# mravanelli/pytorch-kaldi

Hardware: AMD Instinct MI355X
Metric: train_frames_per_sec (higher is better)
Workload: dtype bf16

## Files before the change

include/pk_amd.h:

```cpp
#ifndef PK_AMD_H
#define PK_AMD_H

#include <stdint.h>

#ifdef __cplusplus
extern "C" {
#endif

#define PK_PREC_F32 0
#define PK_PREC_BF16 1

#define PK_ACT_LINEAR 0
#define PK_ACT_RELU 1
#define PK_ACT_TANH 2
#define PK_ACT_SIGMOID 3
#define PK_ACT_LEAKY_RELU 4
#define PK_ACT_ELU 5

#define PK_CELL_LIGRU 0
#define PK_CELL_RNN 1
#define PK_CELL_LSTM 2
#define PK_CELL_GRU 3
#define PK_CELL_MINGRU 4

// ... 152 lines not shown
                         float mask_scalar, const float* ln_gamma, float ln_eps, const float* Y, const float* S,
                         const float* LNS, const float* dY, uint16_t* dGb, int64_t g_pitch, int prefilled, float* lnwork,
                         float* dln_gamma, float* dln_beta);
unsigned pk_persist2_error_count(void);
void pk_persist2_error_reset(void);

int pk_conv1d_pool_fwd(void* stream, const float* x, const float* w, const float* bias, int B, int Cin, int L,
                       int Cout, int K, int pool, float* y, int32_t* argmax, float* work);
int64_t pk_conv_fwd_work_floats(int Cin, int Cout, int K);
int64_t pk_conv_partial_floats(int B, int Cin, int L, int Cout, int K, int pool);
int pk_conv1d_pool_bwd(void* stream, const float* x, const float* w, const float* dy, const int32_t* argmax, int B,
                       int Cin, int L, int Cout, int K, int pool, float* dw, float* dbias, float* dx,
                       float* partial);

int pk_rmsprop_step(void* stream, float* p, const float* g, float* square_avg, int64_t n, float lr, float alpha,
                    float eps, float weight_decay);
int pk_sgd_step(void* stream, float* p, const float* g, float* momentum_buf, int64_t n, float lr, float momentum,
                float weight_decay, int first_step);
int pk_adam_step(void* stream, float* p, const float* g, float* exp_avg, float* exp_avg_sq, float* max_exp_avg_sq,
                 int64_t n, float lr, float beta1, float beta2, float eps, float weight_decay, int step);
int pk_fused_step(void* stream, int kind, float* p, float* g, float* s0, float* s1, float* s2, int64_t n, float lr, float h0,
                  float h1, float h2, float weight_decay, int step, int zero_grad, const int64_t* segs, int nseg,
                  uint16_t* shadow);

unsigned pk_persist_error_count(void);
void pk_persist_error_reset(void);

int pk_linear_bn_act_bf16_covers(int64_t M, int64_t N, int64_t K);
int pk_linear_bn_act_bf16(void* stream, int M, int N, int K, const uint16_t* xb, int64_t ldx, const uint16_t* wb, int64_t ldw,
                          const float* bias, const float* gamma, const float* beta, float eps, float momentum,
                          float* running_mean, float* running_var, int act, const float* mask, float* z, float* a,
                          float* y, uint16_t* yb, int64_t ldyb, float* mean, float* var);
int pk_gemm_bf16_small_splitk(int M, int N, int K);
int pk_linear_bn_act_bf16_sk(void* stream, int M, int N, int K, const uint16_t* xb, int64_t ldx, const uint16_t* wb,
                             int64_t ldw, const float* bias, const float* gamma, const float* beta, float eps,
                             float momentum, float* running_mean, float* running_var, int act, const float* mask,
                             float* z, float* a, float* y, uint16_t* yb, int64_t ldyb, float* mean, float* var,
                             int splitk, float* ws);
int pk_conv1d_pool_dgrad(void* stream, const float* w, const float* dy, const int32_t* argmax, int B, int Cin, int L, int Cout,
                         int K, int pool, float* dx, float* work);
int pk_conv_bf16_covers(int Cin, int Cout, int K, int pool);
int64_t pk_conv_bf16_work_floats(int B, int Cin, int L, int Cout, int K, int pool, int backward);
int pk_conv1d_pool_fwd_bf16(void* stream, const float* x, const float* w, const float* bias, int B, int Cin, int L, int Cout,
                            int K, int pool, float* y, int32_t* argmax, float* work);
int pk_conv1d_pool_bwd_bf16(void* stream, const float* x, const float* w, const float* dy, const int32_t* argmax, int B,
                            int Cin, int L, int Cout, int K, int pool, float* dw, float* dx, float* work);
// ... 21 lines not shown
```

pytorch-kaldi_amd/_lib.py:

```python
import ctypes
import os
import re
import threading

HERE = os.path.dirname(os.path.abspath(__file__))
LIB_PATH = os.path.join(HERE, "lib", "libpk_amd.so")
HEADER = os.path.join(HERE, "..", "include", "pk_amd.h")

_lock = threading.Lock()
_lib = None

c_void_p, c_int, c_float, c_double, c_int64 = ctypes.c_void_p, ctypes.c_int, ctypes.c_float, ctypes.c_double, ctypes.c_int64
P = c_void_p

SIGNATURES = {
    "pk_version": (c_int, []),
    "pk_last_error": (ctypes.c_char_p, []),
    "pk_num_cu": (c_int, []),
    "pk_gemm": (c_int, [P, c_int, c_int, c_int, c_int, c_float, P, c_int64, c_int64, P, c_int64, c_int64, c_float, P,
                        c_int64, P, c_int, P]),
    "pk_gemm_f32_set_form": (None, [c_int]),
    "pk_gemm_bf16_tile_m": (c_int, [c_int]),
    "pk_gemm_bf16_auto_splitk": (c_int, [c_int, c_int, c_int]),
    "pk_gemm_bf16_set_tile": (None, [c_int]),
# ... 76 lines not shown
    "pk_persist2_set_lstm_waves": (None, [c_int]),
    "pk_rec_helper_set_mode": (None, [c_int]),
    "pk_rec_helper_get_mode": (c_int, []),
    "pk_persist2_get_lstm_waves": (c_int, []),
    "pk_persist2_error_count": (ctypes.c_uint, []),
    "pk_persist2_error_reset": (None, []),
    "pk_conv1d_pool_fwd": (c_int, [P, P, P, P, c_int, c_int, c_int, c_int, c_int, c_int, P, P, P]),
    "pk_conv_fwd_work_floats": (c_int64, [c_int, c_int, c_int]),
    "pk_conv_partial_floats": (c_int64, [c_int, c_int, c_int, c_int, c_int, c_int]),
    "pk_conv1d_pool_bwd": (c_int, [P, P, P, P, P, c_int, c_int, c_int, c_int, c_int, c_int, P, P, P, P]),
    "pk_ark_open": (P, [ctypes.c_char_p, c_int64]),
    "pk_ark_close": (None, [P]),
    "pk_ark_next": (c_int, [P, c_int, ctypes.c_char_p, c_int, ctypes.POINTER(c_int64), ctypes.POINTER(c_int64)]),
    "pk_ark_read": (c_int, [P, P]),
    "pk_ark_skip": (c_int, [P]),
    "pk_ivec_next": (c_int, [P, ctypes.c_char_p, c_int, ctypes.POINTER(c_int64)]),
    "pk_ivec_read": (c_int, [P, P]),
    "pk_context_window": (c_int, [P, c_int64, c_int64, c_int, c_int, P]),
    "pk_mean_var_norm": (c_int, [P, c_int64, c_int64]),
    "pk_rmsprop_step": (c_int, [P, P, P, P, c_int64, c_float, c_float, c_float, c_float]),
    "pk_sgd_step": (c_int, [P, P, P, P, c_int64, c_float, c_float, c_float, c_int]),
    "pk_adam_step": (c_int, [P, P, P, P, P, P, c_int64, c_float, c_float, c_float, c_float, c_float, c_int]),
    "pk_fused_step": (c_int, [P, c_int, P, P, P, P, P, c_int64, c_float, c_float, c_float, c_float, c_float, c_int, c_int, P, c_int, P]),
    "pk_persist_error_count": (ctypes.c_uint, []),
    "pk_persist_error_reset": (None, []),
    "pk_linear_bn_act_bf16_covers": (c_int, [c_int64, c_int64, c_int64]),
    "pk_linear_bn_act_bf16": (c_int, [P, c_int, c_int, c_int, P, c_int64, P, c_int64, P, P, P, c_float, c_float, P, P, c_int, P,
                                      P, P, P, P, c_int64, P, P]),
    "pk_gemm_bf16_small_splitk": (c_int, [c_int, c_int, c_int]),
    "pk_linear_bn_act_bf16_sk": (c_int, [P, c_int, c_int, c_int, P, c_int64, P, c_int64, P, P, P, c_float, c_float, P, P, c_int, P,
                                         P, P, P, P, c_int64, P, P, c_int, P]),
    "pk_selftest_mfma": (c_int, [P, ctypes.POINTER(c_int)]),
    "pk_selftest_permlane": (c_int, [P, ctypes.POINTER(c_int)]),
    "pk_selftest_dpp_row_sum": (c_int, [P, ctypes.POINTER(c_int)]),
    "pk_selftest_cu_hog": (c_int, [P, c_int, c_int, P]),
}


def declared_symbols():
    with open(HEADER) as f:
        text = re.sub(r"/\*.*?\*/", "", f.read(), flags=re.S)
    return sorted(set(re.findall(r"\b(pk_[a-z0-9_]+)\s*\(", text)))


class PkError(RuntimeError):
    pass
# ... 199 lines not shown
```

pytorch-kaldi_amd/csrc/pk_optim.hip:

```cpp
#include "pk_common.h"

namespace {

__global__ void rmsprop_kernel(float* __restrict__ p, const float* __restrict__ g, float* __restrict__ sq, long n, float lr,
                               float alpha, float eps, float wd) {
    for (long i = blockIdx.x * (long)blockDim.x + threadIdx.x; i < n; i += (long)gridDim.x * blockDim.x) {
        float gv = g[i];
        const float pv = p[i];
        if (wd != 0.f) gv += wd * pv;
        const float s = alpha * sq[i] + (1.f - alpha) * gv * gv;
        sq[i] = s;
        p[i] = pv - lr * gv / (sqrtf(s) + eps);
    }
}

__global__ void sgd_kernel(float* __restrict__ p, const float* __restrict__ g, float* __restrict__ buf, long n, float lr,
                           float momentum, float wd, int first) {
    for (long i = blockIdx.x * (long)blockDim.x + threadIdx.x; i < n; i += (long)gridDim.x * blockDim.x) {
        float gv = g[i];
        const float pv = p[i];
        if (wd != 0.f) gv += wd * pv;
        if (momentum != 0.f) {
            const float b = first ? gv : momentum * buf[i] + gv;
            buf[i] = b;
// ... 3 lines not shown
    }
}

__global__ void adam_kernel(float* __restrict__ p, const float* __restrict__ g, float* __restrict__ m, float* __restrict__ v,
                            float* __restrict__ vmax, long n, float lr, float beta1, float beta2, float eps, float wd,
                            float bc1, float bc2s) {
    for (long i = blockIdx.x * (long)blockDim.x + threadIdx.x; i < n; i += (long)gridDim.x * blockDim.x) {
        float gv = g[i];
        const float pv = p[i];
        if (wd != 0.f) gv += wd * pv;
        const float mv = beta1 * m[i] + (1.f - beta1) * gv;
        float vv = beta2 * v[i] + (1.f - beta2) * gv * gv;
        m[i] = mv;
        v[i] = vv;
        if (vmax != nullptr) {
            vv = fmaxf(vmax[i], vv);
            vmax[i] = vv;
        }
        const float denom = sqrtf(vv) / bc2s + eps;
        p[i] = pv - (lr / bc1) * (mv / denom);
    }
}

template <int KIND>
__global__ void fused_step_kernel(float* __restrict__ p, float* __restrict__ g, float* __restrict__ s0, float* __restrict__ s1,
                                  float* __restrict__ s2, long n, float lr, float h0, float h1, float h2, float wd, float bc1,
                                  float bc2s, int first, int zero_grad, const long* __restrict__ segs, int nseg,
                                  unsigned short* __restrict__ shadow) {
    for (long i = 4 * (blockIdx.x * (long)blockDim.x + threadIdx.x); i < n; i += 4 * (long)gridDim.x * blockDim.x) {
        f32x4 gv = *reinterpret_cast<const f32x4*>(g + i);
        f32x4 pv = *reinterpret_cast<const f32x4*>(p + i);
        if (wd != 0.f) {
#pragma unroll
            for (int e = 0; e < 4; ++e) gv[e] += wd * pv[e];
        }
        if (KIND == 0) {
            f32x4 sq = *reinterpret_cast<const f32x4*>(s0 + i);
#pragma unroll
            for (int e = 0; e < 4; ++e) {
                sq[e] = h0 * sq[e] + (1.f - h0) * gv[e] * gv[e];
                pv[e] = pv[e] - lr * gv[e] / (sqrtf(sq[e]) + h1);
            }
            *reinterpret_cast<f32x4*>(s0 + i) = sq;
        } else if (KIND == 1) {
            if (h0 != 0.f) {
                f32x4 b = *reinterpret_cast<const f32x4*>(s0 + i);
#pragma unroll
// ... 7 lines not shown
            for (int e = 0; e < 4; ++e) pv[e] = pv[e] - lr * gv[e];
        } else {
            f32x4 m = *reinterpret_cast<const f32x4*>(s0 + i), v = *reinterpret_cast<const f32x4*>(s1 + i);
            f32x4 vm = v;
#pragma unroll
            for (int e = 0; e < 4; ++e) {
                m[e] = h0 * m[e] + (1.f - h0) * gv[e];
                v[e] = h1 * v[e] + (1.f - h1) * gv[e] * gv[e];
                vm[e] = v[e];
            }
            *reinterpret_cast<f32x4*>(s0 + i) = m;
            *reinterpret_cast<f32x4*>(s1 + i) = v;
            if (s2 != nullptr) {
                const f32x4 old = *reinterpret_cast<const f32x4*>(s2 + i);
#pragma unroll
                for (int e = 0; e < 4; ++e) vm[e] = fmaxf(old[e], v[e]);
                *reinterpret_cast<f32x4*>(s2 + i) = vm;
            }
#pragma unroll
            for (int e = 0; e < 4; ++e) pv[e] = pv[e] - (lr / bc1) * (m[e] / (sqrtf(vm[e]) / bc2s + h2));
        }
        *reinterpret_cast<f32x4*>(p + i) = pv;
        if (zero_grad) *reinterpret_cast<f32x4*>(g + i) = f32x4{0.f, 0.f, 0.f, 0.f};
        if (nseg > 0) {
            int lo = 0, hi = nseg;
            while (hi - lo > 1) {
                const int mid = (lo + hi) >> 1;
                if (segs[5 * mid] <= i) lo = mid;
                else hi = mid;
            }
            const long off = segs[5 * lo], rows = segs[5 * lo + 1], cols = segs[5 * lo + 2], pitch = segs[5 * lo + 3], soff = segs[5 * lo + 4];
            const long rel = i - off;
            if (rel >= 0 && rel < rows * cols) {
                const long row = rel / cols, col = rel - row * cols;
                uint2 pk;
                pk.x = pk_pack_bf2(pv[0], pv[1]);
                pk.y = pk_pack_bf2(pv[2], pv[3]);
                *reinterpret_cast<uint2*>(shadow + soff + row * pitch + col) = pk;
            }
        }
    }
}

inline int blocks_for(long n) {
    long b = (n + 255) / 256;
    if (b > 4096) b = 4096;
    if (b < 1) b = 1;
// ... 13 lines not shown

extern "C" int pk_sgd_step(void* stream, float* p, const float* g, float* momentum_buf, int64_t n, float lr,
                           float momentum, float weight_decay, int first_step) {
    if (n == 0) return 0;
    PK_REQUIRE(momentum == 0.f || momentum_buf != nullptr, "pk_sgd_step: momentum needs a buffer");
    hipLaunchKernelGGL(sgd_kernel, dim3(blocks_for(n)), dim3(256), 0, pk_stream(stream), p, g, momentum_buf, (long)n, lr,
                       momentum, weight_decay, first_step);
    PK_LAUNCH_CHECK();
    return 0;
}

extern "C" int pk_adam_step(void* stream, float* p, const float* g, float* exp_avg, float* exp_avg_sq, float* max_exp_avg_sq,
                            int64_t n, float lr, float beta1, float beta2, float eps, float weight_decay, int step) {
    if (n == 0) return 0;
    PK_REQUIRE(step >= 1 && exp_avg != nullptr && exp_avg_sq != nullptr, "pk_adam_step: step counts from 1 and needs both moments");
    const float bc1 = 1.f - powf(beta1, (float)step);
    const float bc2s = sqrtf(1.f - powf(beta2, (float)step));
    hipLaunchKernelGGL(adam_kernel, dim3(blocks_for(n)), dim3(256), 0, pk_stream(stream), p, g, exp_avg, exp_avg_sq,
                       max_exp_avg_sq, (long)n, lr, beta1, beta2, eps, weight_decay, bc1, bc2s);
    PK_LAUNCH_CHECK();
    return 0;
}

extern "C" int pk_fused_step(void* stream, int kind, float* p, float* g, float* s0, float* s1, float* s2, int64_t n, float lr,
                             float h0, float h1, float h2, float weight_decay, int step, int zero_grad, const int64_t* segs,
                             int nseg, uint16_t* shadow) {
    if (n == 0) return 0;
    PK_REQUIRE(kind >= 0 && kind <= 2 && step >= 1, "pk_fused_step: kind 0..2, step counts from 1");
    PK_REQUIRE((n & 3) == 0 && (((uintptr_t)p | (uintptr_t)g | (uintptr_t)s0 | (uintptr_t)s1 | (uintptr_t)s2) & 15) == 0,
               "pk_fused_step: n and the buffers must be multiples of 4 elements / 16-byte aligned");
    PK_REQUIRE(kind != 0 || s0 != nullptr, "pk_fused_step: RMSprop needs its square average");
    PK_REQUIRE(kind != 1 || h0 == 0.f || s0 != nullptr, "pk_fused_step: momentum needs a buffer");
    PK_REQUIRE(kind != 2 || (s0 != nullptr && s1 != nullptr), "pk_fused_step: Adam needs both moments");
    PK_REQUIRE(nseg == 0 || (segs != nullptr && shadow != nullptr && ((uintptr_t)shadow & 7) == 0), "pk_fused_step: null segment table / copy");
    const float bc1 = kind == 2 ? 1.f - powf(h0, (float)step) : 1.f;
    const float bc2s = kind == 2 ? sqrtf(1.f - powf(h1, (float)step)) : 1.f;
    const dim3 grid(blocks_for(n / 4)), block(256);
    hipStream_t st = pk_stream(stream);
    const long* sg = reinterpret_cast<const long*>(segs);
    if (kind == 0) hipLaunchKernelGGL(fused_step_kernel<0>, grid, block, 0, st, p, g, s0, s1, s2, (long)n, lr, h0, h1, h2, weight_decay, bc1, bc2s, 0, zero_grad, sg, nseg, (unsigned short*)shadow);
    else if (kind == 1) hipLaunchKernelGGL(fused_step_kernel<1>, grid, block, 0, st, p, g, s0, s1, s2, (long)n, lr, h0, h1, h2, weight_decay, bc1, bc2s, step == 1 ? 1 : 0, zero_grad, sg, nseg, (unsigned short*)shadow);
    else hipLaunchKernelGGL(fused_step_kernel<2>, grid, block, 0, st, p, g, s0, s1, s2, (long)n, lr, h0, h1, h2, weight_decay, bc1, bc2s, 0, zero_grad, sg, nseg, (unsigned short*)shadow);
    PK_LAUNCH_CHECK();
    return 0;
}
```

pytorch-kaldi_amd/functional.py:

```python
import ctypes
import os
import weakref

import torch

from . import _lib

PREC = {"fp32": 0, "bf16": 1}
ACT = {"linear": 0, "relu": 1, "tanh": 2, "sigmoid": 3, "leaky_relu": 4, "elu": 5}
CELL = {"liGRU": 0, "RNN": 1, "LSTM": 2, "GRU": 3, "minimalGRU": 4}
REC_STEPWISE, REC_PERSISTENT = 0, 1


class _Settings:

    def __init__(self):
        self.precision = os.environ.get("PK_PRECISION", "fp32")
        self.rec_algo = os.environ.get("PK_REC_ALGO", "auto")
        self.mask_rng = os.environ.get("PK_MASK_RNG", "device")
        assert self.mask_rng in ("reference", "reference_host", "device"), self.mask_rng
        self.wgrad_side = _lib.experiment("wgrad_side", "1") != "0"
        self.self_fill = _lib.experiment("rec_self_fill", "1") != "0"
        self.side_late = _lib.experiment("side_late", "1") != "0"
        self.side_cus = _lib.experiment("side_cus", "0") != "0"
# ... 281 lines not shown

def _up(n, m):
    return (n + m - 1) // m * m


def weight_bf16(w):
    sh = getattr(w, "_pk_shadow", None)
    if sh is not None:
        view, version, alive, flat_version = sh
        if alive() is not None:
            owner = getattr(w, "_pk_owner", None)
            owner = owner() if owner is not None else None
            fv = owner.flat._version if owner is not None else flat_version
            if w._version == version and fv == flat_version:
                return view
            cvt_bf16(w.detach(), out=view)
            w._pk_shadow = (view, w._version, alive, fv)
            return view
    owner = getattr(w, "_pk_owner", None)
    owner = owner() if owner is not None else None
    if owner is not None and w.is_contiguous():
        owner.want_shadow(w)
    return cvt_bf16(w.contiguous())


def cvt_bf16(x2, nseg=1, seglen=None, segpad=None, out=None):
    lib = _lib.load()
    rows, cols = x2.shape
    if seglen is None:
        nseg, seglen = 1, cols
    if segpad is None:
        segpad = _up(seglen, 8)
    assert nseg * seglen == cols and x2.stride(1) == 1
    pitch = _up(nseg * segpad, 64)
    if out is None:
        out = torch.empty(rows, pitch, device=x2.device, dtype=torch.bfloat16)
    assert tuple(out.shape) == (rows, pitch) and out.dtype == torch.bfloat16 and out.is_contiguous()
    _lib.check(lib.pk_cvt_bf16(_stream(), _p(x2), x2.stride(0), rows, nseg, seglen, segpad, _p(out), pitch),
               "pk_cvt_bf16")
    return out


_SMALL_SPLITK = _lib.experiment("small_splitk", "1") != "0"


def gemm_bf16(M, N, K, A, lda, a_kc, B, ldb, b_kc, C, ldc, alpha=1.0, beta=0.0, bias=None, splitk=1):
# ... 245 lines not shown
            wp = ctx.wparam
            sk = _splitk(_tiles(N, K), M)
            if M >= 4096 and wp is not None and wp.is_contiguous() and side_targets_any_ok([wp]):
                side_launch(lambda: gemm(N, K, M, dy2, 1, ldy, x2, x2.stride(0), 1, wp.grad, K, beta=1.0, splitk=sk), (dy2, x2), [wp],
                            defer=True)
            else:
                dw = _new(N, K, like=dy2)
                gemm(N, K, M, dy2, 1, ldy, x2, x2.stride(0), 1, dw, K, splitk=sk)
        if ctx.has_bias and ctx.needs_input_grad[2]:
            db = colsum(dy2)
        return dx, dw, db


class _DxShare:
    on = _lib.experiment("head_dx_share", "1") != "0"
    epoch = 0
    epoch_fwd = 0
    table = {}
    alias = None
    cat = {}
    wcat = {}


def _cat_register(key, ctx_id, N, wb, M):
    if not (_DxShare.on and _lib.experiment("head_dx_cat", "1") != "0" and M >= 4096):
        return
    c = _DxShare.cat.get(key)
    if c is None or c["epoch"] != _DxShare.epoch_fwd:
        c = _DxShare.cat[key] = {"epoch": _DxShare.epoch_fwd, "heads": [], "width": 0, "dz": None, "done": set()}
        for k in [k for k, v in _DxShare.cat.items() if v["epoch"] != _DxShare.epoch_fwd]:
            del _DxShare.cat[k]
    c["heads"].append({"id": ctx_id, "N": N, "off": c["width"], "wb": wb})
    c["width"] += _up(N, 64)


def _cat_slot(ctx, M):
    key = getattr(ctx, "dx_share", None)
    c = _DxShare.cat.get(key) if key is not None else None
    if c is None or len(c["heads"]) < 2:
        return None
    pitches = {h["wb"].shape[1] for h in c["heads"]}
    mine = [h for h in c["heads"] if h["id"] == id(ctx)]
    if len(pitches) != 1 or len(mine) != 1 or id(ctx) in c["done"]:
        return None
    if c["dz"] is None:
        c["dz"] = torch.empty(M, c["width"], device=c["heads"][0]["wb"].device, dtype=torch.bfloat16)
    return c, mine[0]


def _cat_finish(key, g):
    c = _DxShare.cat.get(key)
    if c is None or not c["done"] or c["dz"] is None:
        return g
    heads, dz = c["heads"], c["dz"]
    for h in heads:
        if h["id"] not in c["done"]:
            dz[:, h["off"]:h["off"] + _up(h["N"], 64)].zero_()
    wkey = tuple((h["wb"].data_ptr(), h["N"], h["off"]) for h in heads)
    wc = _DxShare.wcat.get(wkey)
    pitch = heads[0]["wb"].shape[1]
    if wc is None:
        _DxShare.wcat.clear()
        wc = _DxShare.wcat[wkey] = torch.zeros(c["width"], pitch, device=dz.device, dtype=torch.bfloat16)
    for h in heads:
        wc[h["off"]:h["off"] + h["N"]].copy_(h["wb"])
    M, K = c["dims"]
    dx2 = _new(M, K, like=dz)
    gemm_bf16(M, K, c["width"], dz, dz.shape[1], 1, wc, pitch, 0, dx2, K)
    del _DxShare.cat[key]
    dx = dx2.view(c["in_shape"])
    return dx if g is None else dx.add_(g)


class _ShareIn(torch.autograd.Function):
    @staticmethod
    def forward(ctx, x):
        ctx.set_materialize_grads(False)
        ctx.key = _dx_share_key(x)
        return x.view_as(x)

    @staticmethod
    def backward(ctx, g):
        if _DxShare.cat:
            g = _cat_finish(ctx.key, g)
        _DxShare.table.clear()
        _DxShare.alias = None
        return g

# ... 115 lines not shown
        db = _new(N, like=y)
        _lib.check(lib.pk_logsoftmax_bwd_bf16(_stream(), _p(dy2), _p(y), M, N, _p(dzb), ldb, _p(part), _p(db)),
                   "pk_logsoftmax_bwd_bf16")
        dx, dw = _linear_bwd_bf16(ctx, dzb, xb, wb, y)
        return dx, dw, (db if ctx.has_bias and ctx.needs_input_grad[2] else None), None, None, None, None


def linear_log_softmax_ok(x, weight):
    return bf16_mode() and x.dim() == 2 and weight.shape[0] <= 2048


def linear_log_softmax(x, weight, bias=None):
    with torch.no_grad():
        w = weight.contiguous()
        x2 = _rows2d(x)
        tw = input_twin(x2)
        wb_plain = weight_bf16(weight)
        if tw is None:
            xb, xseg, wb = _cvt_bf16_shared(x2), None, wb_plain
        elif tw[1][0] == 1 and tw[0].shape[1] == wb_plain.shape[1]:
            xb, xseg, wb = tw[0], None, wb_plain
        else:
            xb, xseg = tw
            wb = cvt_bf16(w, *xseg)
            assert wb.shape[1] == xb.shape[1]
    _DxShare.epoch += 1
    _DxShare.table.clear()
    _DxShare.epoch_fwd = _DxShare.epoch
    xs = _head_input(x)
    y, amax = LinearLogSoftmaxFn.apply(xs, weight if weight.is_contiguous() else w, bias, xb, wb, wb_plain, xseg)
    y._pk_head = (xs, weight, bias, xb, wb_plain, xseg, y._version, amax)
    return y


class HeadNllFn(torch.autograd.Function):

    @staticmethod
    def forward(ctx, x, weight, bias, y, lab, xb, wb, xseg, ignore_index, amax=None):
        lib = _lib.load()
        ctx.set_materialize_grads(False)
        ctx.xseg = xseg
        M, N = y.shape
        lab = lab.contiguous()
        out4 = _new(4, like=y)
        loss = torch.empty((), device=y.device, dtype=torch.float32)
        part = _new(int(lib.pk_nll_err_partial_floats(M)), like=y)
        if amax is not None and _lib.experiment("head_argmax", "1") != "0":
            _lib.check(lib.pk_nll_err_fwd_argmax(_stream(), _p(y), _p(lab), _p(amax), int(ignore_index), M, N, _p(part), _p(out4),
                                                 _p(loss), _p(label_check_counter(y.device))), "pk_nll_err_fwd_argmax")
        else:
            _lib.check(lib.pk_nll_err_fwd(_stream(), _p(y), _p(lab), int(ignore_index), M, N, _p(part), _p(out4), _p(loss),
                                          _p(label_check_counter(y.device))), "pk_nll_err_fwd")
        ctx.save_for_backward(xb, wb, y, lab, out4)
        ctx.dx_share = _dx_share_key(x) if (_DxShare.on and x.is_contiguous()) else None
        if ctx.dx_share is not None and x.requires_grad:
            _cat_register(ctx.dx_share, id(ctx), N, wb, M)
        ctx.dims = (M, N, x.shape[-1])
        ctx.has_bias = bias is not None
        ctx.in_shape = x.shape
        ctx.wparam = weight if isinstance(weight, torch.nn.Parameter) else None
        ctx.ignore_index = int(ignore_index)
        ctx.mark_non_differentiable(out4)
        return loss, out4

    @staticmethod
    def backward(ctx, dloss, _d4):
        lib = _lib.load()
        if dloss is None:
            return (None,) * 10
        xb, wb, y, lab, out4 = ctx.saved_tensors
        M, N, K = ctx.dims
        dl = dloss.contiguous().float()
        ldb = _up(N, 64)
        part = _new(int(lib.pk_logsoftmax_bwd_bf16_partial_floats(M, N)), like=y)
        db = _new(N, like=y)
        cnt = ctypes.c_void_p(out4.data_ptr() + 8)
        cat = _cat_slot(ctx, M) if ctx.needs_input_grad[0] else None
        if cat is not None:
            dz, off = cat[0]["dz"], cat[1]["off"]
# ... 798 lines not shown
            torch.cuda.current_stream().wait_stream(_Prefill.stream)


class RecLayerPerfFn(torch.autograd.Function):

    @staticmethod
    def forward(ctx, x, xb_in, Wcat, bcat, Ucat, gamma, beta, running_mean, running_var, mask, cfg, edge=None):
        ctx.set_materialize_grads(False)
        _need_gpu(x, Wcat, bcat, Ucat, gamma, beta, mask)
        lib = _lib.load()
        cell, act, H, bidir, use_bn, training, eps, momentum, mask_scalar, xseg = cfg[:10]
        ctx.wparams, ctx.uparams = (cfg[10], cfg[11]) if len(cfg) > 10 else (None, None)
        ctx.side_w, ctx.side_u = (bool(cfg[12]), bool(cfg[13])) if len(cfg) > 13 else (False, False)
        ctx.affine = cfg[15] if len(cfg) > 15 else None
        T, B, D = x.shape
        G = lib.pk_rec_num_gates(CELL[cell])
        NS = lib.pk_rec_num_saved(CELL[cell])
        ndir = 2 if bidir else 1
        TB, GH = T * B, G * H
        Wcat = Wcat.contiguous()
        Ucat = Ucat.contiguous()
        if xb_in is None:
            xseg = None
            xb, Wb, K = cvt_bf16(_rows2d(x)), cvt_bf16(Wcat), D
        else:
            nseg, seglen, segpad = xseg
            assert nseg * seglen == D and xb_in.shape[0] == TB
            xb, Wb, K = xb_in, cvt_bf16(Wcat, nseg, seglen, segpad), nseg * segpad
            assert Wb.shape[1] == xb.shape[1]
        Hp = _up(H, 8)
        Yb = torch.empty(TB, _up(ndir * Hp, 64), device=x.device, dtype=torch.bfloat16)
        two_phase = cell in ("GRU", "minimalGRU")
        self_fill = settings.self_fill and lib.pk_rec_self_fill(CELL[cell]) == 1
        dGb = None
        if any(ctx.needs_input_grad) and not self_fill:
            dGb = torch.empty(ndir * TB, _up(G * Hp, 64), device=x.device, dtype=torch.bfloat16)
        Xb = torch.empty_like(Yb) if two_phase else None
        fill = _Prefill()
        if not self_fill:
            fill.start(Yb, Xb, dGb)
        P = _new(TB, GH, like=Wcat)
        mean = var = None
        bn_bufs = cfg[14] if len(cfg) > 14 else None
        pscale = pshift = None
        if use_bn and training and bn_bufs is not None:
            mean, var, pscale, pshift = gemm_bf16_bn_stats(TB, GH, K, xb, xb.shape[1], 1, Wb, Wb.shape[1], 1, P, GH, gates=(
                gamma, beta, eps, H, bn_bufs[0], bn_bufs[1], bn_bufs[2], momentum, ndir * TB))
        elif use_bn and training:
            mean, var = gemm_bf16_bn_stats(TB, GH, K, xb, xb.shape[1], 1, Wb, Wb.shape[1], 1, P, GH)
        else:
            gemm_bf16(TB, GH, K, xb, xb.shape[1], 1, Wb, Wb.shape[1], 1, P, GH)
# ... 116 lines not shown
            sk = _splitk_bf(_tiles_bf(GH, Kx), TB)
            if gview is not None and xseg is None:
                gemm_bf16(GH, Kx, TB, dPb, dPb.shape[1], 0, xb, xb.shape[1], 0, gview, Kx, beta=1.0, splitk=sk)
                return
            gemm_bf16(GH, Kx, TB, dPb, dPb.shape[1], 0, xb, xb.shape[1], 0, dWp, Kx, splitk=sk)
            if gview is not None:
                nseg, seglen, segpad = xseg
                with torch.no_grad():
                    for s_ in range(nseg):
                        gview[:, s_ * seglen:(s_ + 1) * seglen].add_(dWp[:, s_ * segpad:s_ * segpad + seglen])
                return
            if xseg is None:
                dW = dWp
            else:
                nseg, seglen, segpad = xseg
                dW = torch.cat([dWp[:, s_ * segpad:s_ * segpad + seglen] for s_ in range(nseg)], 1)
            if side_w:
                _accumulate_rows(ctx.wparams, [dW[g * H:(g + 1) * H] for g in range(G)])

        if side_w and not late:
            side_launch(do_dW, (dPb, xb, dWp), ctx.wparams)
        dx = None
        if ctx.needs_input_grad[0]:
            Wb2 = Wb if xseg is None else cvt_bf16(Wcat)
            dx = _new(TB, D, like=dY)
            gemm_bf16(TB, D, GH, dPb, dPb.shape[1], 1, Wb2, Wb2.shape[1], 0, dx, D)
            dx = dx.view(T, B, D)
        if late:
            free = 0
            if settings.side_cus:
                held = int(lib.pk_rec_plan_cus(ndir * B, H))
                free = max(int(lib.pk_num_cu()) - held, 0) if held > 0 else 0
            if side_u:
                side_launch(_sized_for(free, do_dU), (Y, S, Yb, dGb, Xb, dU), ctx.uparams)
            if side_w:
                side_launch(_sized_for(free, do_dW), (dPb, xb, dWp), ctx.wparams)
        if not side_w:
            do_dW()
        return dx, None, (None if side_w else dW), dbias, (None if side_u else dU), dgamma, dbeta, None, None, None, None, None


CONV_BF16_DEFAULT = "1"


def conv_bf16_mode():
    return os.environ.get("PK_CONV_BF16", CONV_BF16_DEFAULT)

# ... 68 lines not shown
```

pytorch-kaldi_amd/optim.py:

```python
import ctypes
import os
import weakref

import torch

from . import _lib


def _stream():
    return ctypes.c_void_p(torch.cuda.current_stream().cuda_stream)


class FlatParams:
    def __init__(self, module, align=64):
        self.module = module
        self.params = [p for p in module.parameters()]
        dev = self.params[0].device
        unused = {id(p) for p in module.pk_unused_parameters()} if hasattr(module, "pk_unused_parameters") else set()
        self.unused = [id(p) in unused for p in self.params]
        index = {id(p): i for i, p in enumerate(self.params)}
        units, placed = [], set()
        if hasattr(module, "pk_flat_groups") and _lib.experiment("flat_groups", "1") != "0":
            for grp in module.pk_flat_groups():
                ids = [index[id(q)] for q in grp if id(q) in index and id(q) not in unused and index[id(q)] not in placed]
# ... 9 lines not shown
            off = (off + align - 1) // align * align
            for i in ids:
                self.offsets[i] = off
                off += self.params[i].numel()
        off = (off + align - 1) // align * align
        self.n_active = off
        for i, p in enumerate(self.params):
            if self.unused[i]:
                self.offsets[i] = off
                off += (p.numel() + align - 1) // align * align
        self.numel = off
        self.flat = torch.zeros(off, device=dev, dtype=torch.float32)
        self.grad = torch.zeros(off, device=dev, dtype=torch.float32)
        with torch.no_grad():
            for p, o in zip(self.params, self.offsets):
                n = p.numel()
                self.flat[o:o + n].copy_(p.detach().reshape(-1))
                p.data = self.flat[o:o + n].view(p.shape)
                p.grad = self.grad[o:o + n].view(p.shape)
                p._pk_flat = True
                p._pk_owner = weakref.ref(self)
        self._index = {id(p): i for i, p in enumerate(self.params)}
        self._clean = False
        self._shadow_req = set()
        self._shadow_have = ()
        self.shadow = self.shadow_segs = None

    def want_shadow(self, p):
        i = self._index.get(id(p))
        if (i is not None and not self.unused[i] and p.dim() == 2 and p.shape[1] % 4 == 0 and self.offsets[i] % 4 == 0
                and p.is_cuda):
            self._shadow_req.add(i)

    def invalidate_shadows(self):
        for p in self.params:
            sh = getattr(p, "_pk_shadow", None)
            if sh is not None:
                p._pk_shadow = (sh[0], -1, sh[2], -1)

    def build_shadows(self):
        from . import functional as F_
        want = tuple(sorted(self._shadow_req, key=lambda i: self.offsets[i]))
        if want == self._shadow_have:
            return
        rows = []
        soff = 0
        for i in want:
            p = self.params[i]
            pitch = (p.shape[1] + 63) // 64 * 64
            rows.append((self.offsets[i], p.shape[0], p.shape[1], pitch, soff))
            soff += p.shape[0] * pitch
        self.shadow = torch.zeros(max(soff, 8), device=self.flat.device, dtype=torch.bfloat16)
        self.shadow_segs = torch.tensor(rows, dtype=torch.int64, device=self.flat.device).reshape(-1, 5)
        self._shadow_have = want
        for i, (_o, r, c, pitch, so) in zip(want, rows):
            p = self.params[i]
            view = self.shadow[so:so + r * pitch].view(r, pitch)
            F_.cvt_bf16(p.detach(), out=view)
            p._pk_shadow = (view, p._version, weakref.ref(self.shadow), self.flat._version)

    def zero_grad(self):
        from .functional import join_side
        join_side()
        if self._clean:
            self._clean = False
        else:
            self.grad.zero_()
        for p, o in zip(self.params, self.offsets):
            if p.grad is None or p.grad.data_ptr() != self.grad.data_ptr() + 4 * o:
                p.grad = self.grad[o:o + p.numel()].view(p.shape)


def _flat_mark_dirty(self):
    self._clean = False


FlatParams.mark_dirty = _flat_mark_dirty


class FusedOptimizer:

    _STATE_KEYS = {"rmsprop": ("square_avg",), "sgd": ("momentum_buffer",),
# ... 29 lines not shown
        return next(iter(self.bufs.values()), None)

    def zero_grad(self):
        self.flat.zero_grad()

    def step(self):
        if not self.flat.flat.is_cuda:
            raise _lib.PkError("fused optimizer step runs on the GPU only (no CPU fallback)")
        from .functional import join_side
        join_side()
        lib = _lib.load()
        lr = float(self.param_groups[0]["lr"])
        f = self.flat
        ptr = lambda k: self.bufs[k].data_ptr() if k in self.bufs else None
        if f.n_active % 4 == 0 and _lib.experiment("fused_step", "1") != "0":
            if f._shadow_req and not torch.cuda.is_current_stream_capturing():
                f.build_shadows()
            nseg = len(f._shadow_have)
            zero = bool(self.zero_in_step) and _lib.experiment("opt_zero_in_step", "1") != "0"
            kind = {"rmsprop": 0, "sgd": 1, "adam": 2}[self.kind]
            h = {"rmsprop": (self.alpha, self.eps, 0.0), "sgd": (self.momentum, 0.0, 0.0),
                 "adam": (self.betas[0], self.betas[1], self.eps)}[self.kind]
            s0 = ptr("square_avg") if kind == 0 else ptr("momentum_buffer") if kind == 1 else ptr("exp_avg")
            rc = lib.pk_fused_step(_stream(), kind, f.flat.data_ptr(), f.grad.data_ptr(), s0, ptr("exp_avg_sq"),
                                   ptr("max_exp_avg_sq"), f.n_active, lr, h[0], h[1], h[2], self.weight_decay, self.steps + 1,
                                   int(zero), f.shadow_segs.data_ptr() if nseg else None, nseg,
                                   f.shadow.data_ptr() if nseg else None)
            _lib.check(rc, "fused optimizer step")
            f._clean = zero
            self.steps += 1
            return
        if self.kind == "rmsprop":
            rc = lib.pk_rmsprop_step(_stream(), f.flat.data_ptr(), f.grad.data_ptr(), ptr("square_avg"), f.n_active, lr,
                                     self.alpha, self.eps, self.weight_decay)
        elif self.kind == "sgd":
            rc = lib.pk_sgd_step(_stream(), f.flat.data_ptr(), f.grad.data_ptr(), ptr("momentum_buffer"), f.n_active, lr,
                                 self.momentum, self.weight_decay, int(self.steps == 0))
        else:
            rc = lib.pk_adam_step(_stream(), f.flat.data_ptr(), f.grad.data_ptr(), ptr("exp_avg"), ptr("exp_avg_sq"),
                                  ptr("max_exp_avg_sq"), f.n_active, lr, self.betas[0], self.betas[1], self.eps,
                                  self.weight_decay, self.steps + 1)
        _lib.check(rc, "fused optimizer step")
        self.steps += 1

    def _torch_twin(self):
        import torch.optim as optim
        ps = self.flat.params
        lr = float(self.param_groups[0]["lr"])
        if self.kind == "rmsprop":
            return optim.RMSprop(ps, lr=lr, alpha=self.alpha, eps=self.eps, weight_decay=self.weight_decay)
# ... 75 lines not shown
```

Measured before the change: 3.793 million.

## Keep segmented bf16 weight copies refreshed by the fused optimizer step

Extends the optimizer's bf16 shadow-weight mechanism to multi-parameter, segment-padded layouts such as concatenated gate weights, head dx-cat buffers and segmented linear weights. The fused step kernel now writes the updated fp32 weights straight into each registered bf16 copy through a per-copy segment table. Forward and backward passes can then reuse these copies instead of running a cvt_bf16 conversion kernel each iteration. In exchange the optimizer kernel does more address arithmetic and scattered stores, and the version-tracking bookkeeping becomes more complex.

Result: no change. 3.786 million (-0.2%).

```diff
diff --git a/include/pk_amd.h b/include/pk_amd.h
--- a/include/pk_amd.h
+++ b/include/pk_amd.h
@@ -198,6 +198,9 @@
 int pk_fused_step(void* stream, int kind, float* p, float* g, float* s0, float* s1, float* s2, int64_t n, float lr, float h0,
                   float h1, float h2, float weight_decay, int step, int zero_grad, const int64_t* segs, int nseg,
                   uint16_t* shadow);
+int pk_fused_step_copies(void* stream, int kind, float* p, float* g, float* s0, float* s1, float* s2, int64_t n, float lr,
+                         float h0, float h1, float h2, float weight_decay, int step, int zero_grad, const int64_t* segs,
+                         int nseg);
 
 unsigned pk_persist_error_count(void);
 void pk_persist_error_reset(void);
diff --git a/pytorch-kaldi_amd/_lib.py b/pytorch-kaldi_amd/_lib.py
--- a/pytorch-kaldi_amd/_lib.py
+++ b/pytorch-kaldi_amd/_lib.py
@@ -122,6 +122,7 @@
     "pk_sgd_step": (c_int, [P, P, P, P, c_int64, c_float, c_float, c_float, c_int]),
     "pk_adam_step": (c_int, [P, P, P, P, P, P, c_int64, c_float, c_float, c_float, c_float, c_float, c_int]),
     "pk_fused_step": (c_int, [P, c_int, P, P, P, P, P, c_int64, c_float, c_float, c_float, c_float, c_float, c_int, c_int, P, c_int, P]),
+    "pk_fused_step_copies": (c_int, [P, c_int, P, P, P, P, P, c_int64, c_float, c_float, c_float, c_float, c_float, c_int, c_int, P, c_int]),
     "pk_persist_error_count": (ctypes.c_uint, []),
     "pk_persist_error_reset": (None, []),
     "pk_linear_bn_act_bf16_covers": (c_int, [c_int64, c_int64, c_int64]),
diff --git a/pytorch-kaldi_amd/csrc/pk_optim.hip b/pytorch-kaldi_amd/csrc/pk_optim.hip
--- a/pytorch-kaldi_amd/csrc/pk_optim.hip
+++ b/pytorch-kaldi_amd/csrc/pk_optim.hip
@@ -49,7 +49,55 @@
     }
 }
 
-template <int KIND>
+__device__ __forceinline__ unsigned copy_index(unsigned rel, unsigned cols, unsigned seglen, unsigned segpad, unsigned pitch,
+                                               long* row_out) {
+    const unsigned row = rel / cols, col = rel - row * cols;
+    const unsigned sg = col / seglen;
+    *row_out = (long)row * pitch;
+    return sg * segpad + (col - sg * seglen);
+}
+
+__device__ __forceinline__ void refresh_copies(const long* __restrict__ segs, int nseg, long i, const f32x4 pv) {
+    int lo = 0, hi = nseg;
+    while (hi - lo > 1) {
+        const int mid = (lo + hi) >> 1;
+        if (segs[8 * mid] <= i) lo = mid;
+        else hi = mid;
+    }
+    const long off = segs[8 * lo];
+    for (int s = lo; s >= 0 && segs[8 * s] == off; --s) {
+        const long* sg = segs + 8 * s;
+        const long total = sg[1] * sg[2], rel = i - off;
+        if (rel < 0 || rel >= total) break;
+        const unsigned cols = (unsigned)sg[2], seglen = (unsigned)sg[3], segpad = (unsigned)sg[4], pitch = (unsigned)sg[5];
+        unsigned short* dst = reinterpret_cast<unsigned short*>(sg[6]);
+        long r;
+        if (((cols | seglen) & 3) == 0) {
+            const unsigned c = copy_index((unsigned)rel, cols, seglen, segpad, pitch, &r);
+            uint2 pk;
+            pk.x = pk_pack_bf2(pv[0], pv[1]);
+            pk.y = pk_pack_bf2(pv[2], pv[3]);
+            *reinterpret_cast<uint2*>(dst + r + c) = pk;
+        } else if (((cols | seglen) & 1) == 0) {
+            const unsigned c0 = copy_index((unsigned)rel, cols, seglen, segpad, pitch, &r);
+            *reinterpret_cast<unsigned*>(dst + r + c0) = pk_pack_bf2(pv[0], pv[1]);
+            if (rel + 2 < total) {
+                const unsigned c1 = copy_index((unsigned)rel + 2, cols, seglen, segpad, pitch, &r);
+                *reinterpret_cast<unsigned*>(dst + r + c1) = pk_pack_bf2(pv[2], pv[3]);
+            }
+        } else {
+#pragma unroll
+            for (int e = 0; e < 4; ++e) {
+                if (rel + e < total) {
+                    const unsigned c = copy_index((unsigned)rel + e, cols, seglen, segpad, pitch, &r);
+                    dst[r + c] = pk_f2bf(pv[e]);
+                }
+            }
+        }
+    }
+}
+
+template <int KIND, int WIDE>
 __global__ void fused_step_kernel(float* __restrict__ p, float* __restrict__ g, float* __restrict__ s0, float* __restrict__ s1,
                                   float* __restrict__ s2, long n, float lr, float h0, float h1, float h2, float wd, float bc1,
                                   float bc2s, int first, int zero_grad, const long* __restrict__ segs, int nseg,
@@ -103,7 +151,9 @@
         }
         *reinterpret_cast<f32x4*>(p + i) = pv;
         if (zero_grad) *reinterpret_cast<f32x4*>(g + i) = f32x4{0.f, 0.f, 0.f, 0.f};
-        if (nseg > 0) {
+        if (WIDE) {
+            if (nseg > 0) refresh_copies(segs, nseg, i, pv);
+        } else if (nseg > 0) {
             int lo = 0, hi = nseg;
             while (hi - lo > 1) {
                 const int mid = (lo + hi) >> 1;
@@ -163,9 +213,11 @@
     return 0;
 }
 
-extern "C" int pk_fused_step(void* stream, int kind, float* p, float* g, float* s0, float* s1, float* s2, int64_t n, float lr,
-                             float h0, float h1, float h2, float weight_decay, int step, int zero_grad, const int64_t* segs,
-                             int nseg, uint16_t* shadow) {
+namespace {
+
+template <int WIDE>
+int fused_step(void* stream, int kind, float* p, float* g, float* s0, float* s1, float* s2, int64_t n, float lr, float h0, float h1,
+               float h2, float weight_decay, int step, int zero_grad, const int64_t* segs, int nseg, uint16_t* shadow) {
     if (n == 0) return 0;
     PK_REQUIRE(kind >= 0 && kind <= 2 && step >= 1, "pk_fused_step: kind 0..2, step counts from 1");
     PK_REQUIRE((n & 3) == 0 && (((uintptr_t)p | (uintptr_t)g | (uintptr_t)s0 | (uintptr_t)s1 | (uintptr_t)s2) & 15) == 0,
@@ -173,15 +225,30 @@
     PK_REQUIRE(kind != 0 || s0 != nullptr, "pk_fused_step: RMSprop needs its square average");
     PK_REQUIRE(kind != 1 || h0 == 0.f || s0 != nullptr, "pk_fused_step: momentum needs a buffer");
     PK_REQUIRE(kind != 2 || (s0 != nullptr && s1 != nullptr), "pk_fused_step: Adam needs both moments");
-    PK_REQUIRE(nseg == 0 || (segs != nullptr && shadow != nullptr && ((uintptr_t)shadow & 7) == 0), "pk_fused_step: null segment table / copy");
+    PK_REQUIRE(nseg >= 0 && (nseg == 0 || (segs != nullptr && (WIDE || (shadow != nullptr && ((uintptr_t)shadow & 7) == 0)))),
+               "pk_fused_step: null segment table / copy");
     const float bc1 = kind == 2 ? 1.f - powf(h0, (float)step) : 1.f;
     const float bc2s = kind == 2 ? sqrtf(1.f - powf(h1, (float)step)) : 1.f;
     const dim3 grid(blocks_for(n / 4)), block(256);
     hipStream_t st = pk_stream(stream);
     const long* sg = reinterpret_cast<const long*>(segs);
-    if (kind == 0) hipLaunchKernelGGL(fused_step_kernel<0>, grid, block, 0, st, p, g, s0, s1, s2, (long)n, lr, h0, h1, h2, weight_decay, bc1, bc2s, 0, zero_grad, sg, nseg, (unsigned short*)shadow);
-    else if (kind == 1) hipLaunchKernelGGL(fused_step_kernel<1>, grid, block, 0, st, p, g, s0, s1, s2, (long)n, lr, h0, h1, h2, weight_decay, bc1, bc2s, step == 1 ? 1 : 0, zero_grad, sg, nseg, (unsigned short*)shadow);
-    else hipLaunchKernelGGL(fused_step_kernel<2>, grid, block, 0, st, p, g, s0, s1, s2, (long)n, lr, h0, h1, h2, weight_decay, bc1, bc2s, 0, zero_grad, sg, nseg, (unsigned short*)shadow);
-    PK_LAUNCH_CHECK();
-    return 0;
-}
+    if (kind == 0) hipLaunchKernelGGL((fused_step_kernel<0, WIDE>), grid, block, 0, st, p, g, s0, s1, s2, (long)n, lr, h0, h1, h2, weight_decay, bc1, bc2s, 0, zero_grad, sg, nseg, (unsigned short*)shadow);
+    else if (kind == 1) hipLaunchKernelGGL((fused_step_kernel<1, WIDE>), grid, block, 0, st, p, g, s0, s1, s2, (long)n, lr, h0, h1, h2, weight_decay, bc1, bc2s, step == 1 ? 1 : 0, zero_grad, sg, nseg, (unsigned short*)shadow);
+    else hipLaunchKernelGGL((fused_step_kernel<2, WIDE>), grid, block, 0, st, p, g, s0, s1, s2, (long)n, lr, h0, h1, h2, weight_decay, bc1, bc2s, 0, zero_grad, sg, nseg, (unsigned short*)shadow);
+    PK_LAUNCH_CHECK();
+    return 0;
+}
+
+}
+
+extern "C" int pk_fused_step(void* stream, int kind, float* p, float* g, float* s0, float* s1, float* s2, int64_t n, float lr,
+                             float h0, float h1, float h2, float weight_decay, int step, int zero_grad, const int64_t* segs,
+                             int nseg, uint16_t* shadow) {
+    return fused_step<0>(stream, kind, p, g, s0, s1, s2, n, lr, h0, h1, h2, weight_decay, step, zero_grad, segs, nseg, shadow);
+}
+
+extern "C" int pk_fused_step_copies(void* stream, int kind, float* p, float* g, float* s0, float* s1, float* s2, int64_t n,
+                                    float lr, float h0, float h1, float h2, float weight_decay, int step, int zero_grad,
+                                    const int64_t* segs, int nseg) {
+    return fused_step<1>(stream, kind, p, g, s0, s1, s2, n, lr, h0, h1, h2, weight_decay, step, zero_grad, segs, nseg, nullptr);
+}
diff --git a/pytorch-kaldi_amd/functional.py b/pytorch-kaldi_amd/functional.py
--- a/pytorch-kaldi_amd/functional.py
+++ b/pytorch-kaldi_amd/functional.py
@@ -327,6 +327,22 @@
     if owner is not None and w.is_contiguous():
         owner.want_shadow(w)
     return cvt_bf16(w.contiguous())
+
+
+def weights_bf16(ws, nseg=1, seglen=None, segpad=None, into=None):
+    if ws is None or len(ws) == 0 or _lib.experiment("weight_copies", "1") == "0":
+        return None
+    owner = getattr(ws[0], "_pk_owner", None)
+    owner = owner() if owner is not None else None
+    if owner is None:
+        return None
+    return owner.copy_of(list(ws), nseg, seglen, segpad, into)
+
+
+def _gates_bf16(wps, Wcat, nseg=1, seglen=None, segpad=None):
+    if wps is None or Wcat.data_ptr() != wps[0].data_ptr() or Wcat.shape[0] != sum(w.shape[0] for w in wps):
+        return None
+    return weights_bf16(wps, nseg, seglen, segpad)
 
 
 def cvt_bf16(x2, nseg=1, seglen=None, segpad=None, out=None):
@@ -618,7 +634,7 @@
     wcat = {}
 
 
-def _cat_register(key, ctx_id, N, wb, M):
+def _cat_register(key, ctx_id, N, wb, M, w=None):
     if not (_DxShare.on and _lib.experiment("head_dx_cat", "1") != "0" and M >= 4096):
         return
     c = _DxShare.cat.get(key)
@@ -626,7 +642,7 @@
         c = _DxShare.cat[key] = {"epoch": _DxShare.epoch_fwd, "heads": [], "width": 0, "dz": None, "done": set()}
         for k in [k for k, v in _DxShare.cat.items() if v["epoch"] != _DxShare.epoch_fwd]:
             del _DxShare.cat[k]
-    c["heads"].append({"id": ctx_id, "N": N, "off": c["width"], "wb": wb})
+    c["heads"].append({"id": ctx_id, "N": N, "off": c["width"], "wb": wb, "w": w})
     c["width"] += _up(N, 64)
 
 
@@ -659,7 +675,9 @@
         _DxShare.wcat.clear()
         wc = _DxShare.wcat[wkey] = torch.zeros(c["width"], pitch, device=dz.device, dtype=torch.bfloat16)
     for h in heads:
-        wc[h["off"]:h["off"] + h["N"]].copy_(h["wb"])
+        rows = wc[h["off"]:h["off"] + h["N"]]
+        if h["w"] is None or rows.shape[1] != h["wb"].shape[1] or weights_bf16([h["w"]], into=rows) is None:
+            rows.copy_(h["wb"])
     M, K = c["dims"]
     dx2 = _new(M, K, like=dz)
     gemm_bf16(M, K, c["width"], dz, dz.shape[1], 1, wc, pitch, 0, dx2, K)
@@ -821,7 +839,9 @@
             xb, xseg, wb = tw[0], None, wb_plain
         else:
             xb, xseg = tw
-            wb = cvt_bf16(w, *xseg)
+            wb = weights_bf16([weight], *xseg)
+            if wb is None:
+                wb = cvt_bf16(w, *xseg)
             assert wb.shape[1] == xb.shape[1]
     _DxShare.epoch += 1
     _DxShare.table.clear()
@@ -853,7 +873,7 @@
         ctx.save_for_backward(xb, wb, y, lab, out4)
         ctx.dx_share = _dx_share_key(x) if (_DxShare.on and x.is_contiguous()) else None
         if ctx.dx_share is not None and x.requires_grad:
-            _cat_register(ctx.dx_share, id(ctx), N, wb, M)
+            _cat_register(ctx.dx_share, id(ctx), N, wb, M, weight if isinstance(weight, torch.nn.Parameter) else None)
         ctx.dims = (M, N, x.shape[-1])
         ctx.has_bias = bias is not None
         ctx.in_shape = x.shape
@@ -1698,11 +1718,15 @@
         Ucat = Ucat.contiguous()
         if xb_in is None:
             xseg = None
-            xb, Wb, K = cvt_bf16(_rows2d(x)), cvt_bf16(Wcat), D
+            xb, Wb, K = cvt_bf16(_rows2d(x)), _gates_bf16(ctx.wparams, Wcat), D
+            if Wb is None:
+                Wb = cvt_bf16(Wcat)
         else:
             nseg, seglen, segpad = xseg
             assert nseg * seglen == D and xb_in.shape[0] == TB
-            xb, Wb, K = xb_in, cvt_bf16(Wcat, nseg, seglen, segpad), nseg * segpad
+            xb, Wb, K = xb_in, _gates_bf16(ctx.wparams, Wcat, nseg, seglen, segpad), nseg * segpad
+            if Wb is None:
+                Wb = cvt_bf16(Wcat, nseg, seglen, segpad)
             assert Wb.shape[1] == xb.shape[1]
         Hp = _up(H, 8)
         Yb = torch.empty(TB, _up(ndir * Hp, 64), device=x.device, dtype=torch.bfloat16)
@@ -1865,7 +1889,9 @@
             side_launch(do_dW, (dPb, xb, dWp), ctx.wparams)
         dx = None
         if ctx.needs_input_grad[0]:
-            Wb2 = Wb if xseg is None else cvt_bf16(Wcat)
+            Wb2 = Wb if xseg is None else _gates_bf16(ctx.wparams, Wcat)
+            if Wb2 is None:
+                Wb2 = cvt_bf16(Wcat)
             dx = _new(TB, D, like=dY)
             gemm_bf16(TB, D, GH, dPb, dPb.shape[1], 1, Wb2, Wb2.shape[1], 0, dx, D)
             dx = dx.view(T, B, D)
diff --git a/pytorch-kaldi_amd/optim.py b/pytorch-kaldi_amd/optim.py
--- a/pytorch-kaldi_amd/optim.py
+++ b/pytorch-kaldi_amd/optim.py
@@ -55,42 +55,102 @@
                 p._pk_owner = weakref.ref(self)
         self._index = {id(p): i for i, p in enumerate(self.params)}
         self._clean = False
-        self._shadow_req = set()
+        self._shadow_req = {}
         self._shadow_have = ()
-        self.shadow = self.shadow_segs = None
+        self._shadow_state = {}
+        self.shadow_segs = self._shadow_keep = None
+
+    def _copy_key(self, ps, nseg, seglen, segpad, ext):
+        idx = tuple(self._index.get(id(p)) for p in ps)
+        if not idx or any(i is None or self.unused[i] for i in idx) or ps[0].dim() != 2:
+            return None
+        cols = ps[0].shape[1]
+        off = self.offsets[idx[0]]
+        for i, p in zip(idx, ps):
+            if p.dim() != 2 or p.shape[1] != cols or not p.is_cuda or self.offsets[i] != off:
+                return None
+            off += p.numel()
+        if seglen is None:
+            nseg, seglen = 1, cols
+        if segpad is None:
+            segpad = (seglen + 7) // 8 * 8
+        if (cols == 0 or nseg * seglen != cols or segpad % 8 or segpad < seglen or self.offsets[idx[0]] % 4
+                or off - self.offsets[idx[0]] >= 2 ** 31):
+            return None
+        return (idx, int(nseg), int(seglen), int(segpad), bool(ext))
+
+    def _copy_span(self, key):
+        idx = key[0]
+        return self.offsets[idx[0]], sum(self.params[i].shape[0] for i in idx), self.params[idx[0]].shape[1]
+
+    def _copy_source(self, key):
+        o, rows, cols = self._copy_span(key)
+        return self.flat[o:o + rows * cols].view(rows, cols)
+
+    def copy_of(self, ps, nseg=1, seglen=None, segpad=None, into=None):
+        from . import functional as F_
+        key = self._copy_key(ps, nseg, seglen, segpad, into is not None)
+        if key is None:
+            return None
+        st = self._shadow_state.get(key)
+        if st is not None and (into is None or (st[0].data_ptr() == into.data_ptr() and st[0].shape == into.shape)):
+            versions = tuple(p._version for p in ps)
+            if st[1] != versions or st[2] != self.flat._version:
+                F_.cvt_bf16(self._copy_source(key), key[1], key[2], key[3], out=st[0])
+                st[1], st[2] = versions, self.flat._version
+            return st[0]
+        if key in self._shadow_req and self._shadow_req[key] is into:
+            return None
+        o, rows, cols = self._copy_span(key)
+        for k2 in self._shadow_req:
+            o2, r2, c2 = self._copy_span(k2)
+            if o < o2 + r2 * c2 and o2 < o + rows * cols and (o, rows * cols) != (o2, r2 * c2):
+                return None
+        pitch = (key[1] * key[3] + 63) // 64 * 64
+        if into is not None and not (into.dtype == torch.bfloat16 and into.is_contiguous() and into.data_ptr() % 16 == 0
+                                     and tuple(into.shape) == (rows, pitch)):
+            return None
+        self._shadow_state.pop(key, None)
+        self._shadow_req[key] = into
+        return None
 
     def want_shadow(self, p):
-        i = self._index.get(id(p))
-        if (i is not None and not self.unused[i] and p.dim() == 2 and p.shape[1] % 4 == 0 and self.offsets[i] % 4 == 0
-                and p.is_cuda):
-            self._shadow_req.add(i)
+        if p.dim() == 2:
+            self.copy_of([p])
 
     def invalidate_shadows(self):
         for p in self.params:
             sh = getattr(p, "_pk_shadow", None)
             if sh is not None:
                 p._pk_shadow = (sh[0], -1, sh[2], -1)
+        for st in self._shadow_state.values():
+            st[1], st[2] = None, -1
 
     def build_shadows(self):
         from . import functional as F_
-        want = tuple(sorted(self._shadow_req, key=lambda i: self.offsets[i]))
-        if want == self._shadow_have:
+        want = sorted(self._shadow_req, key=lambda k: (self.offsets[k[0][0]], k[1:]))
+        for key in want:
+            if key not in self._shadow_state:
+                o, rows, cols = self._copy_span(key)
+                view = self._shadow_req[key]
+                if view is None:
+                    view = torch.zeros(rows, (key[1] * key[3] + 63) // 64 * 64, device=self.flat.device, dtype=torch.bfloat16)
+                F_.cvt_bf16(self._copy_source(key), key[1], key[2], key[3], out=view)
+                ps = [self.params[i] for i in key[0]]
+                self._shadow_state[key] = [view, tuple(p._version for p in ps), self.flat._version]
+                if len(ps) == 1 and key[1] == 1 and not key[4]:
+                    ps[0]._pk_shadow = (view, ps[0]._version, weakref.ref(view), self.flat._version)
+        have = tuple((key, self._shadow_state[key][0].data_ptr()) for key in want)
+        if have == self._shadow_have:
             return
-        rows = []
-        soff = 0
-        for i in want:
-            p = self.params[i]
-            pitch = (p.shape[1] + 63) // 64 * 64
-            rows.append((self.offsets[i], p.shape[0], p.shape[1], pitch, soff))
-            soff += p.shape[0] * pitch
-        self.shadow = torch.zeros(max(soff, 8), device=self.flat.device, dtype=torch.bfloat16)
-        self.shadow_segs = torch.tensor(rows, dtype=torch.int64, device=self.flat.device).reshape(-1, 5)
-        self._shadow_have = want
-        for i, (_o, r, c, pitch, so) in zip(want, rows):
-            p = self.params[i]
-            view = self.shadow[so:so + r * pitch].view(r, pitch)
-            F_.cvt_bf16(p.detach(), out=view)
-            p._pk_shadow = (view, p._version, weakref.ref(self.shadow), self.flat._version)
+        table = []
+        for key in want:
+            o, rows, cols = self._copy_span(key)
+            view = self._shadow_state[key][0]
+            table.append((o, rows, cols, key[2], key[3], view.shape[1], view.data_ptr(), 0))
+        self.shadow_segs = torch.tensor(table, dtype=torch.int64, device=self.flat.device).reshape(-1, 8)
+        self._shadow_have = have
+        self._shadow_keep = [self._shadow_state[key][0] for key in want]
 
     def zero_grad(self):
         from .functional import join_side
@@ -166,10 +226,9 @@
             h = {"rmsprop": (self.alpha, self.eps, 0.0), "sgd": (self.momentum, 0.0, 0.0),
                  "adam": (self.betas[0], self.betas[1], self.eps)}[self.kind]
             s0 = ptr("square_avg") if kind == 0 else ptr("momentum_buffer") if kind == 1 else ptr("exp_avg")
-            rc = lib.pk_fused_step(_stream(), kind, f.flat.data_ptr(), f.grad.data_ptr(), s0, ptr("exp_avg_sq"),
-                                   ptr("max_exp_avg_sq"), f.n_active, lr, h[0], h[1], h[2], self.weight_decay, self.steps + 1,
-                                   int(zero), f.shadow_segs.data_ptr() if nseg else None, nseg,
-                                   f.shadow.data_ptr() if nseg else None)
+            rc = lib.pk_fused_step_copies(_stream(), kind, f.flat.data_ptr(), f.grad.data_ptr(), s0, ptr("exp_avg_sq"),
+                                          ptr("max_exp_avg_sq"), f.n_active, lr, h[0], h[1], h[2], self.weight_decay,
+                                          self.steps + 1, int(zero), f.shadow_segs.data_ptr() if nseg else None, nseg)
             _lib.check(rc, "fused optimizer step")
             f._clean = zero
             self.steps += 1
```
